# pudnax/voidin

Hardware: AMD Instinct MI355X
Metric: M instances culled+compacted/sec (higher is better)
Workload: dtype f32; 1 GPU; configs[2]: 10M synthetic AABB instances, cull + prefix-sum compaction (BASELINE.md §3 distribution, model.rs camera); instances_per_gpu=10000000, instances_total=10000000, n_meshes=16, distribution=baseline, parallelism=single GPU

## Files before the change

voidin_amd/csrc/cull.hip:

```cpp
#include "vd_common.hpp"

#include <math.h>

namespace {

constexpr int kWave = 64;
constexpr int kBlock = 256;
constexpr int kWavesPerBlock = kBlock / kWave;
constexpr int kInstBytes = 144;
constexpr int kSlabBytes = kWave * kInstBytes;
constexpr int kChunksPerLane = kSlabBytes / (kWave * 16);



typedef unsigned int u32x4 __attribute__((ext_vector_type(4)));

struct CullCamera {
    float view[16];
    float frustum[4];
    float znear, zfar;
};

struct MeshRec { float mnx, mny, mnz; unsigned index_count; float mxx, mxy, mxz; unsigned base_index; int vertex_offset; };

// ... 315 lines not shown
        if (lane < n_valid && ((in >> lane) & 1ull)) {
            const MeshRec m = load_mesh(meshes, min(li.mesh, n_mesh - 1u));
            keep = !is_occluded(cam, hz, m, li.T0, li.T1, li.T2, li.T3);
        }
        const unsigned long long b = __ballot(keep);
        if (lane == 0) mask_out[wt] = b;
    }
}

constexpr int kMaskRounds = 16;
template <typename IdT>
__global__ __launch_bounds__(kBlock, 3) void cull_mask_tiled_kernel(CullCamera cam, const VdMeshInfo* __restrict__ meshes,
                                                                     unsigned n_mesh, const VdInstance* __restrict__ inst,
                                                                     unsigned n_inst, vd_u64* __restrict__ mask,
                                                                     IdT* __restrict__ ids_out, unsigned* __restrict__ tile_count,
                                                                     unsigned n_tiles) {
    extern __shared__ __attribute__((aligned(16))) char smem[];
    const unsigned lane = threadIdx.x & 63u, wave = threadIdx.x >> 6;
    constexpr int kIdBytes = kMaskRounds * kWave * (int)sizeof(IdT);
    char* slab = smem + wave * (kSlabBytes + kIdBytes);
    IdT* s_ids = reinterpret_cast<IdT*>(slab + kSlabBytes);
    const unsigned waves_total = gridDim.x * kWavesPerBlock;
    auto valid_at = [&](size_t f) -> unsigned { return f < n_inst ? (unsigned)min((size_t)64, (size_t)n_inst - f) : 0u; };
    u32x4 regs[kChunksPerLane];
    for (unsigned t = blockIdx.x * kWavesPerBlock + wave; t < n_tiles; t += waves_total) {
        const size_t tile_first = (size_t)t * (kWave * kMaskRounds);
        slab_fill<true>(inst, tile_first, valid_at(tile_first), lane, regs);
        constexpr int kIdRows = kIdBytes / (kWave * 16);
        u32x4 old_ids[kIdRows];
        const size_t id_base0 = tile_first * sizeof(IdT);
        const bool full_tile = tile_first + (size_t)kWave * kMaskRounds <= (size_t)n_inst;
        if (full_tile) {
#pragma unroll
            for (int r = 0; r < kIdRows; ++r)
                old_ids[r] = *reinterpret_cast<const u32x4*>(reinterpret_cast<const char*>(ids_out) + id_base0 + (size_t)r * kWave * 16 + lane * 16u);
        }
        vd_u64 my_word = 0;
#pragma unroll 1
        for (int r = 0; r < kMaskRounds; ++r) {
            const size_t first = tile_first + (size_t)r * kWave;
            const unsigned n_valid = valid_at(first);
            slab_store(slab, lane, regs);
            if (r + 1 < kMaskRounds) slab_fill<true>(inst, first + kWave, valid_at(first + kWave), lane, regs);
            vd_wave_lds_sync();
            const LaneInst li = slab_read(slab, lane);
            vd_wave_lds_sync();
            const unsigned mid = min(li.mesh, n_mesh - 1u);
            const MeshRec m = load_mesh(meshes, mid);
            const bool vis = lane < n_valid && is_visible(cam, m, li.T0, li.T1, li.T2, li.T3);
            const unsigned long long b = __ballot(vis);
            if (lane == (unsigned)r) my_word = b;
            s_ids[r * kWave + lane] = (IdT)mid;
        }
        vd_wave_lds_sync();
        const size_t w0 = (size_t)t * kMaskRounds;
        const size_t n_words = ((size_t)n_inst + 63) / 64;
        if (lane < (unsigned)kMaskRounds && w0 + lane < n_words) mask[w0 + lane] = my_word;
        unsigned survivors = (unsigned)__popcll(my_word);
#pragma unroll
        for (int off = kMaskRounds / 2; off > 0; off >>= 1) survivors += __shfl_xor(survivors, off);
        if (lane == 0u) tile_count[t] = survivors;
        const size_t id_base = tile_first * sizeof(IdT);
        const size_t id_end = min((size_t)n_inst, tile_first + (size_t)kWave * kMaskRounds) * sizeof(IdT);
        char* gids = reinterpret_cast<char*>(ids_out);
        if (full_tile) {
#pragma unroll
            for (int r = 0; r < kIdRows; ++r) {
                const unsigned b0 = (unsigned)r * kWave * 16u + lane * 16u;
                const u32x4 nv = *reinterpret_cast<const u32x4*>(reinterpret_cast<const char*>(s_ids) + b0);
                const bool diff = nv.x != old_ids[r].x || nv.y != old_ids[r].y || nv.z != old_ids[r].z || nv.w != old_ids[r].w;
                if (__any(diff)) *reinterpret_cast<u32x4*>(gids + id_base + b0) = nv;
            }
        } else {
            for (unsigned b0 = lane * 16u; b0 < (unsigned)kIdBytes; b0 += kWave * 16u) {
                if (id_base + b0 + 16u <= id_end) {
                    *reinterpret_cast<u32x4*>(gids + id_base + b0) = *reinterpret_cast<const u32x4*>(reinterpret_cast<const char*>(s_ids) + b0);
                } else {
                    for (unsigned q = 0; q < 16u && id_base + b0 + q < id_end; ++q) gids[id_base + b0 + q] = reinterpret_cast<const char*>(s_ids)[b0 + q];
                }
            }
        }
        vd_wave_lds_sync();
    }
}

constexpr int kExpandGroup = 4;
constexpr int kExpandWords = 32;
constexpr int kChunkWords = kWavesPerBlock * kExpandWords;

constexpr int kScanBlock = 1024;
struct ScanState { unsigned done, epoch, pad[2]; };
__global__ __launch_bounds__(kScanBlock) void mask_scan_kernel(const vd_u64* __restrict__ mask, unsigned n_words, unsigned n_chunks,
                                                           vd_u64* chunk_entry, ScanState* state,
                                                           unsigned* __restrict__ out_count) {
    constexpr int kScanWaves = kScanBlock / kWave;
    __shared__ unsigned s_last, s_wave_sum[kScanWaves];
    const unsigned lane = threadIdx.x & 63u, wave = threadIdx.x >> 6;
    const unsigned ep = __hip_atomic_load(&state->epoch, VD_RLX_AGENT);
    const vd_u64 tag = (vd_u64)ep << 32;
    for (unsigned c = blockIdx.x * kScanWaves + wave; c < n_chunks; c += gridDim.x * kScanWaves) {
        const unsigned w = c * kChunkWords + lane;
        unsigned v = (w < n_words ? (unsigned)__popcll(mask[w]) : 0u) + (w + 64u < n_words ? (unsigned)__popcll(mask[w + 64u]) : 0u);
#pragma unroll
        for (int off = 32; off > 0; off >>= 1) v += __shfl_xor(v, off);
        if (lane == 0) __hip_atomic_store(&chunk_entry[c], tag | v, VD_RLX_AGENT);
    }
    __builtin_amdgcn_s_waitcnt(0);
    __syncthreads();
    if (threadIdx.x == 0) s_last = __hip_atomic_fetch_add(&state->done, 1u, VD_RLX_AGENT) == gridDim.x - 1u;
    __syncthreads();
    if (!s_last) return;
    const unsigned per = (n_chunks + kScanBlock - 1) / kScanBlock;
    const unsigned begin = min(threadIdx.x * per, n_chunks), end = min(begin + per, n_chunks);
    bool stuck = false;
    auto entry = [&](unsigned c) -> unsigned {
        vd_u64 e = __hip_atomic_load(&chunk_entry[c], VD_RLX_AGENT);
        unsigned spins = 0;
        while ((e >> 32) != (vd_u64)ep) {
            if (++spins > (1u << 22)) { stuck = true; return 0u; }
            __builtin_amdgcn_s_sleep(1);
            e = __hip_atomic_load(&chunk_entry[c], VD_RLX_AGENT);
        }
        return (unsigned)e;
    };
    unsigned sum = 0;
    for (unsigned c = begin; c < end; ++c) sum += entry(c);
    const bool any_stuck = __syncthreads_or(stuck ? 1 : 0) != 0;
    unsigned incl = sum;
#pragma unroll
    for (int off = 1; off < kWave; off <<= 1) {
        const unsigned t = __shfl_up(incl, off);
        if (lane >= (unsigned)off) incl += t;
    }
    if (lane == kWave - 1u) s_wave_sum[wave] = incl;
    __syncthreads();
    unsigned run = incl - sum;
    for (unsigned w = 0; w < wave; ++w) run += s_wave_sum[w];
    for (unsigned c = begin; c < end; ++c) {
        if (any_stuck) { chunk_entry[c] = tag | 0xffffffffu; continue; }
        const unsigned v = entry(c);
        chunk_entry[c] = tag | run;
        run += v;
    }
    if (threadIdx.x == kScanBlock - 1u) {
        *out_count = any_stuck ? 0xffffffffu : run;
        __hip_atomic_store(&state->done, 0u, VD_RLX_AGENT);
        __hip_atomic_store(&state->epoch, ep + 1u, VD_RLX_AGENT);
    }
}

constexpr int kChunkTiles = kChunkWords / kMaskRounds;

__device__ __forceinline__ unsigned tile_prefix_partial(const unsigned* __restrict__ tile_count, unsigned n_before) {
    constexpr unsigned kBatch = 4;
    unsigned sum = 0;
    for (unsigned i0 = threadIdx.x * 4u; i0 < n_before; i0 += kBatch * kBlock * 4u) {
        u32x4 v[kBatch];
#pragma unroll
        for (unsigned k = 0; k < kBatch; ++k) {
            const unsigned i = i0 + k * kBlock * 4u;
            v[k] = *reinterpret_cast<const u32x4*>(tile_count + (i < n_before ? i : i0));
        }
#pragma unroll
        for (unsigned k = 0; k < kBatch; ++k) {
            const unsigned i = i0 + k * kBlock * 4u;
            sum += (i < n_before ? v[k].x : 0u) + (i + 1u < n_before ? v[k].y : 0u) + (i + 2u < n_before ? v[k].z : 0u) +
                   (i + 3u < n_before ? v[k].w : 0u);
        }
    }
#pragma unroll
    for (int off = 32; off > 0; off >>= 1) sum += __shfl_xor(sum, off);
    return sum;
}

template <typename IdT, bool TAB, bool TILES>
__global__ __launch_bounds__(kBlock) void expand_mask_kernel(const vd_u64* __restrict__ mask, unsigned n_words, unsigned wps,
                                                             unsigned shard_size, unsigned n_total, unsigned first_instance,
                                                             const IdT* __restrict__ mesh_ids,
                                                             const VdMeshInfo* __restrict__ meshes, unsigned n_mesh,
                                                             VdDrawIndexedIndirect* __restrict__ out,
                                                             const vd_u64* __restrict__ chunk_entry,
                                                             const unsigned* __restrict__ tile_count, unsigned* __restrict__ out_count) {
    constexpr int kGroups = kExpandWords / kExpandGroup;
    __shared__ unsigned s_prefix[kWavesPerBlock];
    constexpr unsigned kTab = TAB ? 512 : 1;
    __shared__ unsigned s_tab[kTab][3];
    constexpr int kStageBytes = kExpandGroup * 1280 + 32;
    __shared__ __attribute__((aligned(16))) char s_stage[kWavesPerBlock][kStageBytes];
    const unsigned lane = threadIdx.x & 63u, wave = threadIdx.x >> 6;
    const unsigned chunk = blockIdx.x;
    const unsigned cw0 = chunk * kChunkWords;
    const unsigned w0 = __builtin_amdgcn_readfirstlane(cw0 + wave * kExpandWords);
    unsigned base = 0;
    if (TILES) {
        const unsigned part = tile_prefix_partial(tile_count, chunk * kChunkTiles);
        if (lane == 0) s_prefix[wave] = part;
    } else {
        base = (unsigned)chunk_entry[chunk];
        if (base == 0xffffffffu) return;
    }
    unsigned before = 0;
    if (lane < wave * kExpandWords && cw0 + lane < n_words) before = (unsigned)__popcll(mask[cw0 + lane]);
    if (lane + 64u < wave * kExpandWords && cw0 + 64u + lane < n_words) before += (unsigned)__popcll(mask[cw0 + 64u + lane]);
    vd_u64 my_word = 0;
    if (lane < (unsigned)kExpandWords && w0 + lane < n_words) my_word = mask[w0 + lane];
    auto group_first = [&](unsigned wg, unsigned (&f)[kExpandGroup]) {
        unsigned shard = wg / wps, r = wg - shard * wps;
#pragma unroll
        for (int q = 0; q < kExpandGroup; ++q) {
            f[q] = shard * shard_size + 64u * r;
            if (++r >= wps) { r = 0u; ++shard; }
        }
    };
    unsigned ids[kExpandWords];
#pragma unroll
    for (int g = 0; g < kGroups; ++g) {
        const unsigned wg = w0 + g * kExpandGroup;
        unsigned f[kExpandGroup];
        group_first(wg, f);
#pragma unroll
        for (int q = 0; q < kExpandGroup; ++q) {
            const unsigned idx = f[q] + lane;
            ids[g * kExpandGroup + q] = (wg + q < n_words && idx < n_total) ? (unsigned)mesh_ids[idx] : 0u;
        }
    }
    if (TAB)
        for (unsigned i = threadIdx.x; i < n_mesh; i += kBlock) {
            s_tab[i][0] = meshes[i].index_count; s_tab[i][1] = meshes[i].base_index; s_tab[i][2] = (unsigned)meshes[i].vertex_offset;
        }
#pragma unroll
    for (int off = 32; off > 0; off >>= 1) before += __shfl_xor(before, off);
    base += before;
    __syncthreads();
    if (TILES) {
#pragma unroll
        for (int w = 0; w < kWavesPerBlock; ++w) base += s_prefix[w];
        if (chunk == gridDim.x - 1u && wave == kWavesPerBlock - 1u) {
            unsigned mine = (unsigned)__popcll(my_word);
#pragma unroll
            for (int off = 32; off > 0; off >>= 1) mine += __shfl_xor(mine, off);
            if (lane == 0) *out_count = base + mine;
        }
    }
    char* stage = s_stage[wave];
#pragma unroll
    for (int g = 0; g < kGroups; ++g) {
        const unsigned wg = w0 + g * kExpandGroup;
        vd_u64 m[kExpandGroup];
        unsigned cnt = 0;
#pragma unroll
        for (int q = 0; q < kExpandGroup; ++q) {
            const int k = g * kExpandGroup + q;
            const unsigned lo = __shfl((unsigned)my_word, k), hi = __shfl((unsigned)(my_word >> 32), k);
            m[q] = ((vd_u64)hi << 32) | lo;
            cnt += (unsigned)__popcll(m[q]);
        }
        if (cnt == 0u) continue;
        char* gbase = reinterpret_cast<char*>(out + base);
        const unsigned shift = (unsigned)(reinterpret_cast<uintptr_t>(gbase) & 15u);
        unsigned run = 0;
        unsigned first[kExpandGroup];
        group_first(wg, first);
#pragma unroll
        for (int q = 0; q < kExpandGroup; ++q) {
            unsigned mid = ids[g * kExpandGroup + q];
            if ((m[q] >> lane) & 1ull) {
                mid = min(mid, n_mesh - 1u);
                unsigned* o = reinterpret_cast<unsigned*>(stage + shift + 20u * (run + vd_mbcnt(m[q])));
                if (TAB) { o[0] = s_tab[mid][0]; o[2] = s_tab[mid][1]; o[3] = s_tab[mid][2]; }
                else { o[0] = meshes[mid].index_count; o[2] = meshes[mid].base_index; o[3] = (unsigned)meshes[mid].vertex_offset; }
                o[1] = 1u;
                o[4] = first_instance + first[q] + lane;
            }
            run += (unsigned)__popcll(m[q]);
        }
        vd_wave_lds_sync();
        const unsigned total = shift + 20u * cnt;
        char* g16 = gbase - shift;
        for (unsigned b0 = lane * 16u; b0 < total; b0 += kWave * 16u) {
            if (b0 >= shift && b0 + 16u <= total) {
                *reinterpret_cast<u32x4*>(g16 + b0) = *reinterpret_cast<const u32x4*>(stage + b0);
            } else {
                const unsigned lo_b = b0 > shift ? b0 : shift, hi_b = b0 + 16u < total ? b0 + 16u : total;
                for (unsigned b = lo_b; b < hi_b; b += 4u)
                    *reinterpret_cast<unsigned*>(g16 + b) = *reinterpret_cast<const unsigned*>(stage + b);
            }
        }
        vd_wave_lds_sync();
        base += cnt;
    }
}

template <bool DIRECT, bool TILES>
__global__ __launch_bounds__(kBlock) void expand_mask_u8_kernel(const vd_u64* __restrict__ mask, unsigned n_words, unsigned wps,
                                                                unsigned shard_size, unsigned n_total, unsigned first_instance,
                                                                const unsigned char* __restrict__ mesh_ids,
                                                                const VdMeshInfo* __restrict__ meshes, unsigned n_mesh,
                                                                VdDrawIndexedIndirect* __restrict__ out,
                                                                const vd_u64* __restrict__ chunk_entry,
                                                                const unsigned* __restrict__ tile_count, unsigned* __restrict__ out_count) {
    constexpr int kGroups = kExpandWords / kExpandGroup;
    __shared__ unsigned s_prefix[kWavesPerBlock];
    __shared__ __attribute__((aligned(16))) unsigned s_tab[256][4];
    constexpr int kStageBytes = DIRECT ? 16 : kExpandGroup * 1280 + 32;
    __shared__ __attribute__((aligned(16))) char s_stage[kWavesPerBlock][kStageBytes];
    const unsigned lane = threadIdx.x & 63u;
    const unsigned wave = __builtin_amdgcn_readfirstlane(threadIdx.x >> 6);
    const unsigned chunk = blockIdx.x;
    const unsigned cw0 = chunk * kChunkWords;
    const unsigned w0 = cw0 + wave * kExpandWords;
    unsigned base = 0;
    if (TILES) {
        const unsigned part = tile_prefix_partial(tile_count, chunk * kChunkTiles);
        if (lane == 0) s_prefix[wave] = part;
    } else {
        base = (unsigned)chunk_entry[chunk];
        if (base == 0xffffffffu) return;
    }
    unsigned before = 0;
    if (lane < wave * kExpandWords && cw0 + lane < n_words) before = (unsigned)__popcll(mask[cw0 + lane]);
    if (lane + 64u < wave * kExpandWords && cw0 + 64u + lane < n_words) before += (unsigned)__popcll(mask[cw0 + 64u + lane]);
    vd_u64 my_word = 0;
    if (lane < (unsigned)kExpandWords && w0 + lane < n_words) my_word = mask[w0 + lane];
    unsigned ids[kGroups];
    {
        const unsigned wl = w0 + (lane >> 4);
        unsigned shard = wl / wps, r = wl - shard * wps;
#pragma unroll
        for (int g = 0; g < kGroups; ++g) {
            const unsigned i0 = shard * shard_size + 64u * r + 4u * (lane & 15u);
            ids[g] = (wl + g * kExpandGroup < n_words && i0 < n_total) ? *reinterpret_cast<const unsigned*>(mesh_ids + i0) : 0u;
            r += kExpandGroup;
            if (r >= wps) { r -= wps; ++shard; }
        }
    }
    unsigned s_shard = w0 / wps, s_r = w0 - s_shard * wps;
    unsigned word_first = s_shard * shard_size + 64u * s_r;
    constexpr unsigned PF = DIRECT ? 0u : 32u;
    unsigned pf = 0;
    if (PF > 0) {
        const unsigned pw = (chunk + 8u * PF) * kChunkWords + (threadIdx.x >> 1);
        if (pw < n_words) {
            const unsigned ps = pw / wps;
            const unsigned pi = ps * shard_size + 64u * (pw - ps * wps) + 32u * (threadIdx.x & 1u);
            if (pi + 32u <= n_total) {
                const u32x4 a = *reinterpret_cast<const u32x4*>(mesh_ids + pi), b = *reinterpret_cast<const u32x4*>(mesh_ids + pi + 16u);
                pf = a.x ^ a.w ^ b.x ^ b.w;
            }
            if ((threadIdx.x & 1u) == 0u) pf ^= (unsigned)mask[pw];
        }
    }
    if (threadIdx.x < n_mesh) {
        const VdMeshInfo mi = meshes[threadIdx.x];
        s_tab[threadIdx.x][0] = mi.index_count; s_tab[threadIdx.x][1] = 1u;
        s_tab[threadIdx.x][2] = mi.base_index;  s_tab[threadIdx.x][3] = (unsigned)mi.vertex_offset;
    }
#pragma unroll
    for (int off = 32; off > 0; off >>= 1) before += __shfl_xor(before, off);
    base = __builtin_amdgcn_readfirstlane(base + before);
    __syncthreads();
    if (TILES) {
#pragma unroll
        for (int w = 0; w < kWavesPerBlock; ++w) base += s_prefix[w];
        base = __builtin_amdgcn_readfirstlane(base);
        if (chunk == gridDim.x - 1u && wave == kWavesPerBlock - 1u) {
            unsigned mine = (unsigned)__popcll(my_word);
#pragma unroll
            for (int off = 32; off > 0; off >>= 1) mine += __shfl_xor(mine, off);
            if (lane == 0) *out_count = base + mine;
        }
    }
    const unsigned max_mid = n_mesh - 1u;
    const unsigned inst_lane = first_instance + lane;
    const unsigned id_shift = 8u * (lane & 3u);
    char* stage = s_stage[wave];
#pragma unroll
    for (int g = 0; g < kGroups; ++g) {
        vd_u64 m[kExpandGroup];
        unsigned cnt = 0;
#pragma unroll
        for (int q = 0; q < kExpandGroup; ++q) {
            const int k = g * kExpandGroup + q;
            const unsigned lo = __builtin_amdgcn_readlane((unsigned)my_word, k), hi = __builtin_amdgcn_readlane((unsigned)(my_word >> 32), k);
            m[q] = ((vd_u64)hi << 32) | lo;
            cnt += (unsigned)__popcll(m[q]);
        }
        unsigned wf[kExpandGroup];
#pragma unroll
        for (int q = 0; q < kExpandGroup; ++q) {
            wf[q] = word_first;
            if (++s_r >= wps) { s_r = 0u; ++s_shard; }
            word_first = s_shard * shard_size + 64u * s_r;
        }
        if (cnt == 0u) continue;
        if (DIRECT) {
            unsigned run = base;
#pragma unroll
            for (int q = 0; q < kExpandGroup; ++q) {
                const unsigned v = (unsigned)__shfl((int)ids[g], q * 16 + (int)(lane >> 2));
                const unsigned mid = min((v >> id_shift) & 0xffu, max_mid);
                if (__builtin_amdgcn_inverse_ballot_w64(m[q])) {
                    unsigned* o = reinterpret_cast<unsigned*>(out + (run + vd_mbcnt(m[q])));
                    typedef u32x4 __attribute__((aligned(4))) u32x4_a4;
                    *reinterpret_cast<u32x4_a4*>(o) = *reinterpret_cast<const u32x4*>(s_tab[mid]);
                    o[4] = inst_lane + wf[q];
                }
                run += (unsigned)__popcll(m[q]);
            }
        } else {
            char* gbase = reinterpret_cast<char*>(out + base);
            const unsigned shift = (unsigned)(reinterpret_cast<uintptr_t>(gbase) & 15u);
            unsigned run = 0;
#pragma unroll
            for (int q = 0; q < kExpandGroup; ++q) {
                const unsigned v = (unsigned)__shfl((int)ids[g], q * 16 + (int)(lane >> 2));
                const unsigned mid = min((v >> id_shift) & 0xffu, max_mid);
                if (__builtin_amdgcn_inverse_ballot_w64(m[q])) {
                    unsigned* o = reinterpret_cast<unsigned*>(stage + shift + 20u * (run + vd_mbcnt(m[q])));
                    const u32x4 c = *reinterpret_cast<const u32x4*>(s_tab[mid]);
                    o[0] = c.x; o[1] = c.y; o[2] = c.z; o[3] = c.w;
                    o[4] = inst_lane + wf[q];
                }
                run += (unsigned)__popcll(m[q]);
            }
            vd_wave_lds_sync();
            const unsigned total = shift + 20u * cnt;
            char* g16 = gbase - shift;
            for (unsigned b0 = lane * 16u; b0 < total; b0 += kWave * 16u) {
                if (b0 >= shift && b0 + 16u <= total) {
                    *reinterpret_cast<u32x4*>(g16 + b0) = *reinterpret_cast<const u32x4*>(stage + b0);
                } else {
                    const unsigned lo_b = b0 > shift ? b0 : shift, hi_b = b0 + 16u < total ? b0 + 16u : total;
                    for (unsigned b = lo_b; b < hi_b; b += 4u)
                        *reinterpret_cast<unsigned*>(g16 + b) = *reinterpret_cast<const unsigned*>(stage + b);
                }
            }
            vd_wave_lds_sync();
        }
        base += cnt;
    }
    if (PF > 0 && pf == 0x9e3779b9u && n_mesh == 0u) out[0].instance_count = pf;
}

template <typename IdT>
__global__ __launch_bounds__(kBlock) void emit_from_mask_kernel(const vd_u64* __restrict__ mask, const IdT* __restrict__ mesh_ids,
                                                               const VdMeshInfo* __restrict__ meshes, unsigned n_mesh,
                                                               unsigned n_inst, unsigned first_instance,
                                                               VdDrawIndexedIndirect* __restrict__ out) {
    constexpr unsigned kTab = 512;
    __shared__ __attribute__((aligned(16))) unsigned s_tab[kTab][4];
    const bool tab = n_mesh <= kTab;
    if (tab)
        for (unsigned i = threadIdx.x; i < n_mesh; i += kBlock) {
            s_tab[i][0] = meshes[i].index_count; s_tab[i][1] = 0u;
            s_tab[i][2] = meshes[i].base_index;  s_tab[i][3] = (unsigned)meshes[i].vertex_offset;
        }
    __syncthreads();
    const unsigned n_quads = (n_inst + 3u) / 4u;
    for (unsigned q = blockIdx.x * kBlock + threadIdx.x; q < n_quads; q += gridDim.x * kBlock) {
        const unsigned i0 = q * 4u;
        const unsigned bits = (unsigned)(mask[i0 >> 6] >> (i0 & 63u)) & 15u;
        unsigned mid[4];
#pragma unroll
        for (int k = 0; k < 4; ++k) mid[k] = i0 + k < n_inst ? min((unsigned)mesh_ids[i0 + k], n_mesh - 1u) : 0u;
        unsigned w[20];
#pragma unroll
        for (int k = 0; k < 4; ++k) {
            u32x4 c;
            if (tab) c = *reinterpret_cast<const u32x4*>(s_tab[mid[k]]);
            else { c.x = meshes[mid[k]].index_count; c.z = meshes[mid[k]].base_index; c.w = (unsigned)meshes[mid[k]].vertex_offset; }
            w[5 * k] = c.x; w[5 * k + 1] = (bits >> k) & 1u; w[5 * k + 2] = c.z; w[5 * k + 3] = c.w; w[5 * k + 4] = first_instance + i0 + k;
        }
        unsigned* o = reinterpret_cast<unsigned*>(out + i0);
        if (i0 + 4u <= n_inst) {
#pragma unroll
            for (int k = 0; k < 5; ++k) {
                u32x4 v; v.x = w[4 * k]; v.y = w[4 * k + 1]; v.z = w[4 * k + 2]; v.w = w[4 * k + 3];
                *reinterpret_cast<u32x4*>(o + 4 * k) = v;
            }
        } else {
            for (unsigned k = 0; k < 5u * (n_inst - i0); ++k) o[k] = w[k];
        }
    }
}

__global__ __launch_bounds__(kBlock) void emit_all_u8_kernel(const vd_u64* __restrict__ mask, unsigned n_words, unsigned n_inst,
                                                             unsigned first_instance, const unsigned char* __restrict__ mesh_ids,
                                                             const VdMeshInfo* __restrict__ meshes, unsigned n_mesh,
                                                             VdDrawIndexedIndirect* __restrict__ out) {
    constexpr int kGroups = kExpandWords / kExpandGroup;
    __shared__ __attribute__((aligned(16))) unsigned s_tab[256][4];
    const unsigned lane = threadIdx.x & 63u;
    const unsigned wave = __builtin_amdgcn_readfirstlane(threadIdx.x >> 6);
    const unsigned w0 = (blockIdx.x * kWavesPerBlock + wave) * kExpandWords;
    vd_u64 my_word = 0;
    if (lane < (unsigned)kExpandWords && w0 + lane < n_words) my_word = mask[w0 + lane];
    unsigned ids[kGroups];
#pragma unroll
    for (int g = 0; g < kGroups; ++g) {
        const unsigned i0 = 64u * (w0 + g * kExpandGroup + (lane >> 4)) + 4u * (lane & 15u);
        ids[g] = i0 < n_inst ? *reinterpret_cast<const unsigned*>(mesh_ids + i0) : 0u;
    }
    if (threadIdx.x < n_mesh) {
        const VdMeshInfo mi = meshes[threadIdx.x];
        s_tab[threadIdx.x][0] = mi.index_count; s_tab[threadIdx.x][1] = 0u;
        s_tab[threadIdx.x][2] = mi.base_index;  s_tab[threadIdx.x][3] = (unsigned)mi.vertex_offset;
    }
    __syncthreads();
    const unsigned max_mid = n_mesh - 1u;
    const unsigned id_shift = 8u * (lane & 3u);
#pragma unroll
    for (int g = 0; g < kGroups; ++g) {
#pragma unroll
        for (int q = 0; q < kExpandGroup; ++q) {
            const int k = g * kExpandGroup + q;
            const unsigned lo = __builtin_amdgcn_readlane((unsigned)my_word, k), hi = __builtin_amdgcn_readlane((unsigned)(my_word >> 32), k);
            const vd_u64 m = ((vd_u64)hi << 32) | lo;
            const unsigned v = (unsigned)__shfl((int)ids[g], q * 16 + (int)(lane >> 2));
            const unsigned mid = min((v >> id_shift) & 0xffu, max_mid);
            const unsigned i = 64u * (w0 + (unsigned)k) + lane;
            if (i < n_inst) {
                u32x4 c = *reinterpret_cast<const u32x4*>(s_tab[mid]);
                c.y = (unsigned)(m >> lane) & 1u;
                unsigned* o = reinterpret_cast<unsigned*>(out + i);
                typedef u32x4 __attribute__((aligned(4))) u32x4_a4;
                *reinterpret_cast<u32x4_a4*>(o) = c;
                o[4] = first_instance + i;
            }
        }
    }
}

__global__ __launch_bounds__(kBlock) void mask_to_indices_kernel(const vd_u64* __restrict__ mask, unsigned n_words, unsigned first_instance,
                                                                 unsigned* __restrict__ out, const vd_u64* __restrict__ chunk_entry) {
    const unsigned lane = threadIdx.x & 63u;
    const unsigned wave = __builtin_amdgcn_readfirstlane(threadIdx.x >> 6);
    const unsigned cw0 = blockIdx.x * kChunkWords;
    const unsigned w0 = cw0 + wave * kExpandWords;
    unsigned base = (unsigned)chunk_entry[blockIdx.x];
    if (base == 0xffffffffu) return;
    unsigned before = 0;
    if (lane < wave * kExpandWords && cw0 + lane < n_words) before = (unsigned)__popcll(mask[cw0 + lane]);
    if (lane + 64u < wave * kExpandWords && cw0 + 64u + lane < n_words) before += (unsigned)__popcll(mask[cw0 + 64u + lane]);
    vd_u64 my_word = 0;
    if (lane < (unsigned)kExpandWords && w0 + lane < n_words) my_word = mask[w0 + lane];
#pragma unroll
    for (int off = 32; off > 0; off >>= 1) before += __shfl_xor(before, off);
    base = __builtin_amdgcn_readfirstlane(base + before);
    const unsigned inst_lane = first_instance + 64u * w0 + lane;
#pragma unroll
    for (int k = 0; k < kExpandWords; ++k) {
        const unsigned lo = __builtin_amdgcn_readlane((unsigned)my_word, k), hi = __builtin_amdgcn_readlane((unsigned)(my_word >> 32), k);
        const vd_u64 m = ((vd_u64)hi << 32) | lo;
        if (__builtin_amdgcn_inverse_ballot_w64(m)) out[base + vd_mbcnt(m)] = inst_lane + 64u * (unsigned)k;
        base += (unsigned)__popcll(m);
    }
}

template <typename IdT>
__global__ __launch_bounds__(kBlock) void indices_to_draws_kernel(const unsigned* __restrict__ indices, unsigned n_indices,
                                                                  const IdT* __restrict__ mesh_ids, unsigned n_total,
                                                                  const VdMeshInfo* __restrict__ meshes, unsigned n_mesh,
                                                                  VdDrawIndexedIndirect* __restrict__ out) {
    constexpr unsigned kTab = 512;
    __shared__ __attribute__((aligned(16))) unsigned s_tab[kTab][4];
    const bool tab = n_mesh <= kTab;
    if (tab)
        for (unsigned i = threadIdx.x; i < n_mesh; i += kBlock) {
            s_tab[i][0] = meshes[i].index_count; s_tab[i][1] = 1u;
            s_tab[i][2] = meshes[i].base_index;  s_tab[i][3] = (unsigned)meshes[i].vertex_offset;
        }
    __syncthreads();
    for (unsigned k = blockIdx.x * kBlock + threadIdx.x; k < n_indices; k += gridDim.x * kBlock) {
        const unsigned i = indices[k];
        const unsigned mid = min((unsigned)mesh_ids[min(i, n_total - 1u)], n_mesh - 1u);
        u32x4 c;
        if (tab) c = *reinterpret_cast<const u32x4*>(s_tab[mid]);
        else { c.x = meshes[mid].index_count; c.y = 1u; c.z = meshes[mid].base_index; c.w = (unsigned)meshes[mid].vertex_offset; }
        unsigned* o = reinterpret_cast<unsigned*>(out + k);
        typedef u32x4 __attribute__((aligned(4))) u32x4_a4;
        *reinterpret_cast<u32x4_a4*>(o) = c;
        o[4] = i;
    }
}

static int launch_mask_scan(VdCtx* ctx, const vd_u64* d_mask, unsigned n_words, unsigned* d_out_count, vd_u64** out_entries) {
    const unsigned n_chunks = (n_words + kChunkWords - 1) / kChunkWords;
    const size_t need = sizeof(ScanState) + (size_t)n_chunks * 8;
    if (need > ctx->expand_state_bytes || !ctx->expand_state) {
        int rc = vd_ensure(ctx, &ctx->expand_state, &ctx->expand_state_bytes, need);
        if (rc) return rc;
        VD_HIP_CHECK(ctx, hipMemsetAsync(ctx->expand_state, 0, ctx->expand_state_bytes, ctx->stream));
        VD_HIP_CHECK(ctx, hipMemsetD32Async(reinterpret_cast<hipDeviceptr_t>(reinterpret_cast<char*>(ctx->expand_state) + offsetof(ScanState, epoch)), 1, 1, ctx->stream));
    }
    ScanState* state = reinterpret_cast<ScanState*>(ctx->expand_state);
    vd_u64* entries = reinterpret_cast<vd_u64*>(reinterpret_cast<char*>(ctx->expand_state) + sizeof(ScanState));
    unsigned sblocks = (n_chunks + 15u) / 16u;
    if (sblocks > (unsigned)ctx->num_cus * 2u) sblocks = (unsigned)ctx->num_cus * 2u;
    hipLaunchKernelGGL(mask_scan_kernel, dim3(sblocks), dim3(kScanBlock), 0, ctx->stream, d_mask, n_words, n_chunks, entries, state,
                       d_out_count);
    *out_entries = entries;
    return VD_OK;
}

static int launch_expand(VdCtx* ctx, const vd_u64* d_mask, unsigned n_words, unsigned wps, unsigned shard_size,
                         unsigned n_total, unsigned first_instance, const void* d_ids, unsigned id_bytes,
                         const VdMeshInfo* d_meshes, unsigned n_mesh, VdDrawIndexedIndirect* d_out, unsigned* d_out_count,
                         const unsigned* d_tile_count = nullptr) {
    const unsigned n_chunks = (n_words + kChunkWords - 1) / kChunkWords;
    vd_u64* offsets = nullptr;
    if (!d_tile_count) {
        int rc_scan = launch_mask_scan(ctx, d_mask, n_words, d_out_count, &offsets);
        if (rc_scan) return rc_scan;
    }
    const bool one_shard = wps >= n_words;
    const bool tab = n_mesh <= 512u;
    const bool fast = id_bytes == 1u && n_mesh <= 256u && (one_shard || (shard_size % 4u == 0u && wps >= (unsigned)kExpandGroup)) &&
                      (reinterpret_cast<uintptr_t>(d_ids) & 3u) == 0u;
    if (fast) {
#define VD_EXPAND_U8(D, T)                                                                                                  \
        hipLaunchKernelGGL((expand_mask_u8_kernel<D, T>), dim3(n_chunks), dim3(kBlock), 0, ctx->stream, d_mask, n_words, wps, \
                           shard_size, n_total, first_instance, reinterpret_cast<const unsigned char*>(d_ids), d_meshes,      \
                           n_mesh, d_out, offsets, d_tile_count, d_out_count)
        const bool direct = n_total <= (12u << 20);
        if (d_tile_count) { if (direct) VD_EXPAND_U8(true, true); else VD_EXPAND_U8(false, true); }
        else { if (direct) VD_EXPAND_U8(true, false); else VD_EXPAND_U8(false, false); }
#undef VD_EXPAND_U8
        return VD_OK;
    }
#define VD_EXPAND_T(IdT, T, S)                                                                                             \
    hipLaunchKernelGGL((expand_mask_kernel<IdT, T, S>), dim3(n_chunks), dim3(kBlock), 0, ctx->stream, d_mask, n_words, wps, \
                       shard_size, n_total, first_instance, reinterpret_cast<const IdT*>(d_ids), d_meshes, n_mesh, d_out,    \
                       offsets, d_tile_count, d_out_count)
#define VD_EXPAND(IdT, T) do { if (d_tile_count) VD_EXPAND_T(IdT, T, true); else VD_EXPAND_T(IdT, T, false); } while (0)
    if (id_bytes == 1u) { if (tab) VD_EXPAND(unsigned char, true); else VD_EXPAND(unsigned char, false); }
    else if (id_bytes == 2u) { if (tab) VD_EXPAND(unsigned short, true); else VD_EXPAND(unsigned short, false); }
    else { if (tab) VD_EXPAND(unsigned, true); else VD_EXPAND(unsigned, false); }
#undef VD_EXPAND
#undef VD_EXPAND_T
    return VD_OK;
}

__global__ __launch_bounds__(kBlock) void pad_tail_kernel(VdDrawIndexedIndirect* __restrict__ out,
                                                          const unsigned* __restrict__ count, unsigned n) {
    const unsigned c = *count;
    const size_t begin = (c > n ? (size_t)0 : (size_t)c) * 5u, end = (size_t)n * 5u;
    unsigned* o = reinterpret_cast<unsigned*>(out);
    if (begin >= end) return;
    const size_t gid = (size_t)blockIdx.x * kBlock + threadIdx.x, gsz = (size_t)gridDim.x * kBlock;
    const size_t mis = (reinterpret_cast<uintptr_t>(o + begin) >> 2) & 3u;
    const size_t head = min(end - begin, (4u - mis) & 3u);
    const size_t quads = (end - begin - head) >> 2;
    const size_t tail_first = begin + head + quads * 4u;
    if (gid < head) o[begin + gid] = 0u;
    if (gid < end - tail_first) o[tail_first + gid] = 0u;
    u32x4* q = reinterpret_cast<u32x4*>(o + begin + head);
    const u32x4 z = {0u, 0u, 0u, 0u};
    for (size_t i = gid; i < quads; i += gsz) __builtin_nontemporal_store(z, q + i);
}

constexpr int kCompactPerThread = 8;
constexpr int kCompactTile = kBlock * kCompactPerThread;

__global__ __launch_bounds__(kBlock) void compact_draws_kernel(const VdDrawIndexedIndirect* __restrict__ in, unsigned n,
                                                               VdDrawIndexedIndirect* __restrict__ out,
                                                               unsigned* __restrict__ out_count, vd_u64* tile_state,
                                                               vd_u64* ticket_counter, unsigned n_tiles, unsigned* fault_host) {
    __shared__ unsigned s_ticket, s_epoch, s_wave_total[kWavesPerBlock], s_tile_excl;
    const unsigned lane = threadIdx.x & 63u, wave = threadIdx.x >> 6;
    if (threadIdx.x == 0) s_ticket = vd_take_ticket(ticket_counter, n_tiles, &s_epoch);
    __syncthreads();
    const unsigned tile = s_ticket, epoch = s_epoch;
    if (tile >= n_tiles) return;
    if (tile == 0u && threadIdx.x == 0) { __hip_atomic_store(out_count, VD_SCAN_STUCK, VD_RLX_AGENT); __threadfence(); }
    const size_t wave_first = (size_t)tile * kCompactTile + (size_t)wave * (kWave * kCompactPerThread);
    unsigned long long masks[kCompactPerThread];
    unsigned wave_total = 0;
    const unsigned* in32 = reinterpret_cast<const unsigned*>(in);
#pragma unroll
    for (int r = 0; r < kCompactPerThread; ++r) {
        const size_t i = wave_first + (size_t)r * kWave + lane;
        const bool keep = i < n && in32[i * 5u + 1u] == 1u;
        masks[r] = __ballot(keep);
        wave_total += (unsigned)__popcll(masks[r]);
    }
    if (lane == 0) s_wave_total[wave] = wave_total;
    __syncthreads();
    if (wave == 0) {
        unsigned tile_total = 0;
#pragma unroll
        for (int w = 0; w < kWavesPerBlock; ++w) tile_total += s_wave_total[w];
        const unsigned excl = vd_lookback(tile_state, epoch, tile, tile_total);
        if (lane == 0) {
            s_tile_excl = excl;
            if (tile == n_tiles - 1u) *out_count = vd_scan_final_count(tile_state, epoch, excl, tile_total, fault_host);
        }
    }
    __syncthreads();
    unsigned base = s_tile_excl;
    if (base == VD_SCAN_STUCK) return;
    for (unsigned w = 0; w < wave; ++w) base += s_wave_total[w];
    unsigned* out32 = reinterpret_cast<unsigned*>(out);
#pragma unroll
    for (int r = 0; r < kCompactPerThread; ++r) {
        const unsigned long long mask = masks[r];
        if ((mask >> lane) & 1ull) {
            const size_t i = wave_first + (size_t)r * kWave + lane;
            const size_t d = (size_t)(base + vd_mbcnt(mask)) * 5u;
#pragma unroll
            for (int k = 0; k < 5; ++k) out32[d + k] = in32[i * 5u + k];
        }
        base += (unsigned)__popcll(mask);
    }
}

struct RotZ { float c_pos, s_pos, c_neg, s_neg; };
template <int SRC> __device__ __forceinline__ float quad_bcast(float v) {
    return __int_as_float(__builtin_amdgcn_mov_dpp(__float_as_int(v), SRC * 0x55, 0xf, 0xf, true));
}
__global__ __launch_bounds__(256) void compute_update_kernel(const unsigned* __restrict__ indices, unsigned n_indices,
                                                             VdInstance* __restrict__ inst, unsigned n_inst, RotZ rz, int fix_inverse) {
    const unsigned t = blockIdx.x * 256u + threadIdx.x, k = t >> 2, col = t & 3u;
    const unsigned idx = k < n_indices ? indices[k] : 0xffffffffu;
    const bool live = idx < n_inst;
    float4* t4 = reinterpret_cast<float4*>(inst[live ? idx : 0u].transform);
    float4 v = make_float4(0.0f, 0.0f, 0.0f, 0.0f);
    if (live) v = t4[col];
    const float t14 = quad_bcast<3>(v.z);
    const bool pos = t14 > -15.0f;
    const float c = pos ? rz.c_pos : rz.c_neg, s = pos ? rz.s_pos : rz.s_neg;
    float4 o;
    o.x = ((c * v.x + -s * v.y) + 0.0f * v.z) + 0.0f * v.w;
    o.y = ((s * v.x + c * v.y) + 0.0f * v.z) + 0.0f * v.w;
    o.z = ((0.0f * v.x + 0.0f * v.y) + 1.0f * v.z) + 0.0f * v.w;
    o.w = ((0.0f * v.x + 0.0f * v.y) + 0.0f * v.z) + 1.0f * v.w;
    if (live) t4[col] = o;
    if (fix_inverse) {
        float4* i4 = reinterpret_cast<float4*>(inst[live ? idx : 0u].inv_transform);
        float4 w = make_float4(0.0f, 0.0f, 0.0f, 0.0f);
        if (live) w = i4[col];
        const float4 I0 = make_float4(quad_bcast<0>(w.x), quad_bcast<0>(w.y), quad_bcast<0>(w.z), quad_bcast<0>(w.w));
        const float4 I1 = make_float4(quad_bcast<1>(w.x), quad_bcast<1>(w.y), quad_bcast<1>(w.z), quad_bcast<1>(w.w));
        const float4 I2 = make_float4(quad_bcast<2>(w.x), quad_bcast<2>(w.y), quad_bcast<2>(w.z), quad_bcast<2>(w.w));
        const float4 I3 = make_float4(quad_bcast<3>(w.x), quad_bcast<3>(w.y), quad_bcast<3>(w.z), quad_bcast<3>(w.w));
        const float b0 = col == 0u ? c : (col == 1u ? s : 0.0f);
        const float b1 = col == 0u ? -s : (col == 1u ? c : 0.0f);
        const float b2 = col == 2u ? 1.0f : 0.0f, b3 = col == 3u ? 1.0f : 0.0f;
        float4 r;
        r.x = ((I0.x * b0 + I1.x * b1) + I2.x * b2) + I3.x * b3;
        r.y = ((I0.y * b0 + I1.y * b1) + I2.y * b2) + I3.y * b3;
        r.z = ((I0.z * b0 + I1.z * b1) + I2.z * b2) + I3.z * b3;
        r.w = ((I0.w * b0 + I1.w * b1) + I2.w * b2) + I3.w * b3;
        if (live) i4[col] = r;
    }
}

CullCamera make_cam(const VdCameraUniform* c) {
    CullCamera k;
    memcpy(k.view, c->view, sizeof(k.view));
    memcpy(k.frustum, c->frustum, sizeof(k.frustum));
    k.znear = c->znear;
    k.zfar = c->zfar;
    return k;
}

}

extern "C" {

int vd_cull_emit_dev(VdCtx* ctx, const VdCameraUniform* camera, const VdMeshInfo* d_meshes, uint32_t n_mesh,
                     const VdInstance* d_instances, uint32_t n_inst, VdDrawIndexedIndirect* d_out) {
    VdDeviceGuard vd_guard_(ctx);
    return vd_cull_emit_shard_dev(ctx, camera, d_meshes, n_mesh, d_instances, n_inst, 0u, d_out);
}

static int launch_mask_pass(VdCtx* ctx, const VdCameraUniform* camera, const VdMeshInfo* d_meshes, uint32_t n_mesh,
                            const VdInstance* d_instances, uint32_t n_inst, vd_u64** out_mask, void** out_ids, unsigned* out_id_bytes,
                            unsigned** out_tile_count) {
    const unsigned n_words = (n_inst + 63u) / 64u;
    const unsigned id_bytes = n_mesh <= 256u ? 1u : (n_mesh <= 65536u ? 2u : 4u);
    const unsigned n_mt = (n_inst + kWave * kMaskRounds - 1) / (kWave * kMaskRounds);
    const size_t ids_off = ((size_t)n_words * 8 + 255) & ~(size_t)255;
    const size_t counts_off = (ids_off + (size_t)n_inst * id_bytes + 15) & ~(size_t)15;
    const size_t need = counts_off + (((size_t)n_mt + 3) & ~(size_t)3) * 4 + 512;
    int rc = vd_ensure(ctx, &ctx->scratch, &ctx->scratch_bytes, need);
    if (rc) return rc;
    vd_u64* d_mask = reinterpret_cast<vd_u64*>(ctx->scratch);
    void* d_ids = reinterpret_cast<char*>(ctx->scratch) + ids_off;
    unsigned* d_counts = reinterpret_cast<unsigned*>(reinterpret_cast<char*>(ctx->scratch) + counts_off);
    vd_time_begin(ctx);
    unsigned mb = (n_mt + kWavesPerBlock - 1) / kWavesPerBlock;
    if (mb > (unsigned)ctx->num_cus * 3u) mb = (unsigned)ctx->num_cus * 3u;
#define VD_SPLIT(IdT)                                                                                              \
    hipLaunchKernelGGL(cull_mask_tiled_kernel<IdT>, dim3(mb), dim3(kBlock),                                        \
                       kWavesPerBlock * (kSlabBytes + kMaskRounds * kWave * (int)sizeof(IdT)),                     \
                       ctx->stream, make_cam(camera), d_meshes, n_mesh, d_instances, n_inst, d_mask,               \
                       reinterpret_cast<IdT*>(d_ids), d_counts, n_mt)
    if (id_bytes == 1u) VD_SPLIT(unsigned char);
    else if (id_bytes == 2u) VD_SPLIT(unsigned short);
    else VD_SPLIT(unsigned);
#undef VD_SPLIT
    vd_time_mid(ctx);
    *out_mask = d_mask; *out_ids = d_ids; *out_id_bytes = id_bytes; *out_tile_count = d_counts;
    return VD_OK;
}

int vd_cull_emit_shard_dev(VdCtx* ctx, const VdCameraUniform* camera, const VdMeshInfo* d_meshes, uint32_t n_mesh,
                           const VdInstance* d_instances, uint32_t n_inst, uint32_t first_instance,
                           VdDrawIndexedIndirect* d_out) {
    VdDeviceGuard vd_guard_(ctx);
    if (!ctx) return VD_ERR_INVALID_ARG;
    if (!camera || !d_meshes || n_mesh == 0) VD_FAIL(ctx, VD_ERR_INVALID_ARG, "vd_cull_emit: null camera/meshes or n_mesh == 0");
    if (n_inst == 0) return VD_OK;
    if (!d_instances || !d_out) VD_FAIL(ctx, VD_ERR_INVALID_ARG, "vd_cull_emit: null instances/out");
    if (ctx->option(VD_OPT_CULL_VARIANT, 0) <= 0 && n_inst >= ctx->split_min) {
        vd_u64* d_mask; void* d_ids; unsigned id_bytes; unsigned* d_tile_count;
        int rc = launch_mask_pass(ctx, camera, d_meshes, n_mesh, d_instances, n_inst, &d_mask, &d_ids, &id_bytes, &d_tile_count);
        if (rc) return rc;
        const unsigned quads = (n_inst + 3u) / 4u;
        unsigned eb = (quads + kBlock - 1) / kBlock;
        if (eb > (unsigned)ctx->num_cus * 16u) eb = (unsigned)ctx->num_cus * 16u;
#define VD_EMIT(IdT) hipLaunchKernelGGL(emit_from_mask_kernel<IdT>, dim3(eb), dim3(kBlock), 0, ctx->stream, d_mask,               \
                                        reinterpret_cast<const IdT*>(d_ids), d_meshes, n_mesh, n_inst, first_instance, d_out)
        if (id_bytes == 1u) {
            const unsigned n_words = (n_inst + 63u) / 64u;
            hipLaunchKernelGGL(emit_all_u8_kernel, dim3((n_words + kChunkWords - 1) / kChunkWords), dim3(kBlock), 0, ctx->stream, d_mask,
                               n_words, n_inst, first_instance, reinterpret_cast<const unsigned char*>(d_ids), d_meshes, n_mesh, d_out);
        } else if (id_bytes == 2u) VD_EMIT(unsigned short); else VD_EMIT(unsigned);
#undef VD_EMIT
        vd_time_end(ctx);
        VD_HIP_CHECK(ctx, hipGetLastError());
        return VD_OK;
    }
    const unsigned n_wave_tiles = (n_inst + kWave - 1) / kWave;
    unsigned blocks = (n_wave_tiles + kWavesPerBlock - 1) / kWavesPerBlock;
    const unsigned cap = (unsigned)ctx->num_cus * 4u;
    if (blocks > cap) blocks = cap;
    vd_time_begin(ctx);
    hipLaunchKernelGGL(emit_draws_kernel, dim3(blocks), dim3(kBlock), kWavesPerBlock * kSlabBytes, ctx->stream,
                       make_cam(camera), d_meshes, n_mesh, d_instances, n_inst, d_out, n_wave_tiles, first_instance);
    vd_time_end(ctx);
    VD_HIP_CHECK(ctx, hipGetLastError());
    return VD_OK;
}

int vd_cull_compact_dev(VdCtx* ctx, const VdCameraUniform* camera, const VdMeshInfo* d_meshes, uint32_t n_mesh,
                        const VdInstance* d_instances, uint32_t n_inst, VdDrawIndexedIndirect* d_out,
                        uint32_t* d_out_count, int pad_tail) {
    VdDeviceGuard vd_guard_(ctx);
    return vd_cull_compact_shard_dev(ctx, camera, d_meshes, n_mesh, d_instances, n_inst, 0u, d_out, d_out_count, pad_tail);
}

int vd_cull_compact_shard_dev(VdCtx* ctx, const VdCameraUniform* camera, const VdMeshInfo* d_meshes, uint32_t n_mesh,
                              const VdInstance* d_instances, uint32_t n_inst, uint32_t first_instance,
                              VdDrawIndexedIndirect* d_out, uint32_t* d_out_count, int pad_tail) {
    VdDeviceGuard vd_guard_(ctx);
    if (!ctx) return VD_ERR_INVALID_ARG;
    if (!camera || !d_meshes || n_mesh == 0 || !d_out_count)
        VD_FAIL(ctx, VD_ERR_INVALID_ARG, "vd_cull_compact: null camera/meshes/count or n_mesh == 0");
    if (n_inst == 0) {
        VD_HIP_CHECK(ctx, hipMemsetAsync(d_out_count, 0, 4, ctx->stream));
        return VD_OK;
    }
    if (!d_instances || !d_out) VD_FAIL(ctx, VD_ERR_INVALID_ARG, "vd_cull_compact: null instances/out");
    const int variant = (int)ctx->option(VD_OPT_CULL_VARIANT, 0);
    vd_u64* ticket; vd_u64* states;
    int rc = vd_scan_check_fault(ctx);
    if (rc) return rc;
    if (variant <= 0 && n_inst >= ctx->split_min) {
        vd_u64* d_mask; void* d_ids; unsigned id_bytes; unsigned* d_tile_count;
        rc = launch_mask_pass(ctx, camera, d_meshes, n_mesh, d_instances, n_inst, &d_mask, &d_ids, &id_bytes, &d_tile_count);
        if (rc) return rc;
        const unsigned n_words = (n_inst + 63u) / 64u;
        rc = launch_expand(ctx, d_mask, n_words, n_words, n_inst, n_inst, first_instance, d_ids, id_bytes, d_meshes, n_mesh,
                           d_out, d_out_count, d_tile_count);
        if (rc) return rc;
        vd_time_end(ctx);
        if (pad_tail) {
            unsigned pblocks = (unsigned)ctx->num_cus * 4u;
            hipLaunchKernelGGL(pad_tail_kernel, dim3(pblocks), dim3(kBlock), 0, ctx->stream, d_out, d_out_count, n_inst);
        }
        VD_HIP_CHECK(ctx, hipGetLastError());
        return VD_OK;
    }
#define VD_LAUNCH_COMPACT(R)                                                                                     \
    do {                                                                                                         \
        const unsigned n_tiles = (n_inst + kBlock * (R) - 1) / (kBlock * (R));                                   \
        rc = vd_scan_scratch(ctx, n_tiles, &ticket, &states, true);                                              \
        if (rc) return rc;                                                                                       \
        hipLaunchKernelGGL((cull_compact_kernel<R>), dim3(n_tiles), dim3(kBlock), (compact_lds_bytes<R>()),      \
                           ctx->stream, make_cam(camera), d_meshes, n_mesh, d_instances, n_inst, d_out,          \
                           d_out_count, states, ticket, n_tiles, first_instance, vd_scan_fault_word(ctx));       \
    } while (0)
    const int rounds = variant > 0 ? variant : (n_inst >= (4u << 20) ? 32 : (n_inst >= (5u << 18) ? 16 : (n_inst >= 600000u ? 8 : (n_inst >= 192000u ? 4 : (n_inst >= 48000u ? 2 : 1)))));
    switch (rounds) {
        case 1: VD_LAUNCH_COMPACT(1); break;
        case 2: VD_LAUNCH_COMPACT(2); break;
        case 4: VD_LAUNCH_COMPACT(4); break;
        case 8: VD_LAUNCH_COMPACT(8); break;
        case 16: VD_LAUNCH_COMPACT(16); break;
        default: VD_LAUNCH_COMPACT(32); break;
    }
#undef VD_LAUNCH_COMPACT
    vd_time_end(ctx);
    if (pad_tail) {
        unsigned blocks = (unsigned)ctx->num_cus * 4u;
        hipLaunchKernelGGL(pad_tail_kernel, dim3(blocks), dim3(kBlock), 0, ctx->stream, d_out, d_out_count, n_inst);
    }
    VD_HIP_CHECK(ctx, hipGetLastError());
    return VD_OK;
}

int vd_cull_mask_dev(VdCtx* ctx, const VdCameraUniform* camera, const VdMeshInfo* d_meshes, uint32_t n_mesh,
                     const VdInstance* d_instances, uint32_t n_inst, uint64_t* d_mask) {
    VdDeviceGuard vd_guard_(ctx);
    if (!ctx) return VD_ERR_INVALID_ARG;
    if (!camera || !d_meshes || n_mesh == 0) VD_FAIL(ctx, VD_ERR_INVALID_ARG, "vd_cull_mask: null camera/meshes or n_mesh == 0");
    if (n_inst == 0) return VD_OK;
    if (!d_instances || !d_mask) VD_FAIL(ctx, VD_ERR_INVALID_ARG, "vd_cull_mask: null instances/mask");
    const unsigned n_wave_tiles = (n_inst + kWave - 1) / kWave;
    unsigned blocks = (n_wave_tiles + kWavesPerBlock - 1) / kWavesPerBlock;
    const unsigned cap = (unsigned)ctx->num_cus * 4u;
    if (blocks > cap) blocks = cap;
    vd_time_begin(ctx);
    hipLaunchKernelGGL(cull_mask_kernel<unsigned>, dim3(blocks), dim3(kBlock), kWavesPerBlock * kSlabBytes, ctx->stream, make_cam(camera),
                       d_meshes, n_mesh, d_instances, n_inst, reinterpret_cast<vd_u64*>(d_mask), (unsigned*)nullptr, n_wave_tiles);
    vd_time_end(ctx);
// ... 225 lines not shown
```

Measured before the change: 39700 M instances/s.

## Stage compacted draw commands in LDS and flush full 128-byte lines

The staged (non-direct) expand path now carries a per-wave LDS staging buffer across groups. It writes only whole 128-byte-aligned cache lines to global memory, moves the leftover tail to the start of the buffer, and flushes the remainder once at the end. Previously each group flushed its 20-byte records with a 16-byte-aligned shift, which produced partial-line writes. The direct/staged threshold is also lowered so the 10M-instance config now takes the staged path instead of the direct scatter path. This adds LDS traffic and extra synchronisation, and the unaligned-head and tail handling is intricate.

```diff
diff --git a/voidin_amd/csrc/cull.hip b/voidin_amd/csrc/cull.hip
--- a/voidin_amd/csrc/cull.hip
+++ b/voidin_amd/csrc/cull.hip
@@ -641,7 +641,7 @@
     constexpr int kGroups = kExpandWords / kExpandGroup;
     __shared__ unsigned s_prefix[kWavesPerBlock];
     __shared__ __attribute__((aligned(16))) unsigned s_tab[256][4];
-    constexpr int kStageBytes = DIRECT ? 16 : kExpandGroup * 1280 + 32;
+    constexpr int kStageBytes = DIRECT ? 16 : kExpandGroup * 1280 + 128;
     __shared__ __attribute__((aligned(16))) char s_stage[kWavesPerBlock][kStageBytes];
     const unsigned lane = threadIdx.x & 63u;
     const unsigned wave = __builtin_amdgcn_readfirstlane(threadIdx.x >> 6);
@@ -713,6 +713,10 @@
     const unsigned inst_lane = first_instance + lane;
     const unsigned id_shift = 8u * (lane & 3u);
     char* stage = s_stage[wave];
+    constexpr unsigned kLine = 128u;
+    unsigned pos = (unsigned)(reinterpret_cast<uintptr_t>(out + base) & (kLine - 1u));
+    char* g_line = reinterpret_cast<char*>(out + base) - pos;
+    unsigned lo = pos;
 #pragma unroll
     for (int g = 0; g < kGroups; ++g) {
         vd_u64 m[kExpandGroup];
@@ -720,8 +724,8 @@
 #pragma unroll
         for (int q = 0; q < kExpandGroup; ++q) {
             const int k = g * kExpandGroup + q;
-            const unsigned lo = __builtin_amdgcn_readlane((unsigned)my_word, k), hi = __builtin_amdgcn_readlane((unsigned)(my_word >> 32), k);
-            m[q] = ((vd_u64)hi << 32) | lo;
+            const unsigned mlo = __builtin_amdgcn_readlane((unsigned)my_word, k), mhi = __builtin_amdgcn_readlane((unsigned)(my_word >> 32), k);
+            m[q] = ((vd_u64)mhi << 32) | mlo;
             cnt += (unsigned)__popcll(m[q]);
         }
         unsigned wf[kExpandGroup];
@@ -747,15 +751,13 @@
                 run += (unsigned)__popcll(m[q]);
             }
         } else {
-            char* gbase = reinterpret_cast<char*>(out + base);
-            const unsigned shift = (unsigned)(reinterpret_cast<uintptr_t>(gbase) & 15u);
             unsigned run = 0;
 #pragma unroll
             for (int q = 0; q < kExpandGroup; ++q) {
                 const unsigned v = (unsigned)__shfl((int)ids[g], q * 16 + (int)(lane >> 2));
                 const unsigned mid = min((v >> id_shift) & 0xffu, max_mid);
                 if (__builtin_amdgcn_inverse_ballot_w64(m[q])) {
-                    unsigned* o = reinterpret_cast<unsigned*>(stage + shift + 20u * (run + vd_mbcnt(m[q])));
+                    unsigned* o = reinterpret_cast<unsigned*>(stage + pos + 20u * (run + vd_mbcnt(m[q])));
                     const u32x4 c = *reinterpret_cast<const u32x4*>(s_tab[mid]);
                     o[0] = c.x; o[1] = c.y; o[2] = c.z; o[3] = c.w;
                     o[4] = inst_lane + wf[q];
@@ -763,20 +765,31 @@
                 run += (unsigned)__popcll(m[q]);
             }
             vd_wave_lds_sync();
-            const unsigned total = shift + 20u * cnt;
-            char* g16 = gbase - shift;
-            for (unsigned b0 = lane * 16u; b0 < total; b0 += kWave * 16u) {
-                if (b0 >= shift && b0 + 16u <= total) {
-                    *reinterpret_cast<u32x4*>(g16 + b0) = *reinterpret_cast<const u32x4*>(stage + b0);
-                } else {
-                    const unsigned lo_b = b0 > shift ? b0 : shift, hi_b = b0 + 16u < total ? b0 + 16u : total;
-                    for (unsigned b = lo_b; b < hi_b; b += 4u)
-                        *reinterpret_cast<unsigned*>(g16 + b) = *reinterpret_cast<const unsigned*>(stage + b);
+            pos += 20u * cnt;
+            const unsigned full = pos & ~(kLine - 1u);
+            if (full != 0u) {
+                for (unsigned b0 = lane * 16u; b0 < pos; b0 += kWave * 16u) {
+                    const u32x4 v = *reinterpret_cast<const u32x4*>(stage + b0);
+                    if (b0 >= full) {
+                        *reinterpret_cast<u32x4*>(stage + (b0 - full)) = v;
+                    } else if (b0 >= lo) {
+                        *reinterpret_cast<u32x4*>(g_line + b0) = v;
+                    } else if (b0 + 16u > lo) {
+                        unsigned* gd = reinterpret_cast<unsigned*>(g_line + b0);
+                        if (b0 + 4u >= lo) gd[1] = v.y;
+                        if (b0 + 8u >= lo) gd[2] = v.z;
+                        gd[3] = v.w;
+                    }
                 }
+                vd_wave_lds_sync();
+                g_line += full; pos -= full; lo = 0u;
             }
-            vd_wave_lds_sync();
         }
         base += cnt;
+    }
+    if (!DIRECT && pos > lo) {
+        const unsigned b = lane * 4u;
+        if (b >= lo && b < pos) *reinterpret_cast<unsigned*>(g_line + b) = *reinterpret_cast<const unsigned*>(stage + b);
     }
     if (PF > 0 && pf == 0x9e3779b9u && n_mesh == 0u) out[0].instance_count = pf;
 }
@@ -961,7 +974,7 @@
         hipLaunchKernelGGL((expand_mask_u8_kernel<D, T>), dim3(n_chunks), dim3(kBlock), 0, ctx->stream, d_mask, n_words, wps, \
                            shard_size, n_total, first_instance, reinterpret_cast<const unsigned char*>(d_ids), d_meshes,      \
                            n_mesh, d_out, offsets, d_tile_count, d_out_count)
-        const bool direct = n_total <= (12u << 20);
+        const bool direct = n_total < (3u << 20);
         if (d_tile_count) { if (direct) VD_EXPAND_U8(true, true); else VD_EXPAND_U8(false, true); }
         else { if (direct) VD_EXPAND_U8(true, false); else VD_EXPAND_U8(false, false); }
 #undef VD_EXPAND_U8
```

Measured after the change: 39830 M instances/s (median of 6 runs). No clear change (+0.3%).
